# VainF/Diff-Pruning

Measured on AMD Instinct MI355X. Metric: importance-scored images/sec (UNet fwd+bwd+|w*dL/dw|), higher is better.
Workload: dtype f32

## Files before the change

### diff-pruning_amd/csrc/norm.hip

```cpp
#include <cstdlib>
#include "dp_common.h"

#define GN_CACHE 32
#define GN_MAXCPG 64

struct GnSrc {
    const float* x1; const float* x2; int c_split; long long s1, s2;
};

__device__ __forceinline__ const float* gn_chan_ptr(const GnSrc& s, int n, int c, int HW) {
    return (c < s.c_split) ? s.x1 + (long long)n * s.s1 + (long long)c * HW
                           : s.x2 + (long long)n * s.s2 + (long long)(c - s.c_split) * HW;
}

__global__ __launch_bounds__(256) void gn_fwd_kernel(GnSrc src, const float* __restrict__ gamma, const float* __restrict__ beta,
                                                     int C, int HW, int G, float eps, int silu, float* __restrict__ y,
                                                     long long y_img_stride, float* __restrict__ stats, DpDrop drop) {
    __shared__ float red[4];
    const int n = blockIdx.x / G;
    const int g = blockIdx.x - n * G;
    const int cpg = C / G;
    const int cnt = cpg * HW;
    const long long didx0 = ((drop.n_off + n) * C + (long long)g * cpg) * HW;
    const int tid = threadIdx.x;
// ... 38 lines not shown
    }
    const float var = dp_block_sum_256(q, red) / (float)cnt;
    const float rstd = 1.0f / sqrtf(var + eps);
    if (tid == 0) {
        stats[(long long)blockIdx.x * 2 + 0] = mean;
        stats[(long long)blockIdx.x * 2 + 1] = rstd;
    }
    float* yb = y + (long long)n * y_img_stride + (long long)c_base * HW;
    if (cached) {
#pragma unroll
        for (int i = 0; i < GN_CACHE; ++i) {
            const int e = tid + 256 * i;
            if (e < cnt) {
                const int c = c_base + e / HW;
                float v = (xr[i] - mean) * rstd * gamma[c] + beta[c];
                if (silu) v = dp_silu(v);
                if (drop.thr24) v *= dp_drop1(drop, didx0 + e);
                yb[e] = v;
            }
        }
    } else {
        for (int e = tid; e < cnt; e += 256) {
            const int cl = e / HW;
            const int c = c_base + cl;
            float v = (gn_chan_ptr(src, n, c, HW)[e - cl * HW] - mean) * rstd * gamma[c] + beta[c];
            if (silu) v = dp_silu(v);
            if (drop.thr24) v *= dp_drop1(drop, didx0 + e);
            yb[e] = v;
        }
    }
}

template <int NI>
__global__ __launch_bounds__(256) void gn_fwd_vec4_kernel(GnSrc src, const float* __restrict__ gamma,
                                                          const float* __restrict__ beta, int C, int HW, int G, float eps,
                                                          int silu, float* __restrict__ y, long long y_img_stride,
                                                          float* __restrict__ stats, DpDrop drop) {
    __shared__ float red[4];
    const int n = blockIdx.x / G;
    const int g = blockIdx.x - n * G;
    const int cpg = C / G;
    const int cnt4 = cpg * HW / 4;
    const long long didx0 = ((drop.n_off + n) * C + (long long)g * cpg) * HW;
    const int HW4 = HW / 4;
    const int tid = threadIdx.x;
    constexpr bool cached = NI > 0;
    constexpr int NC = NI > 0 ? NI : 1;
    const int c_base = g * cpg;
    float4 xr[NC];
    float gac[NC], bec[NC];
    float s = 0.f;
    if (cached) {
#pragma unroll
        for (int i = 0; i < NC; ++i) {
            const int e = tid + 256 * i;
            const int ec = e < cnt4 ? e : cnt4 - 1;
            const int cl = ec / HW4;
            xr[i] = reinterpret_cast<const float4*>(gn_chan_ptr(src, n, c_base + cl, HW))[ec - cl * HW4];
            gac[i] = gamma[c_base + cl];
            bec[i] = beta[c_base + cl];
        }
#pragma unroll
        for (int i = 0; i < NC; ++i) {
            if (tid + 256 * i >= cnt4) xr[i] = make_float4(0.f, 0.f, 0.f, 0.f);
            const float4 v = xr[i];
            s += (v.x + v.y) + (v.z + v.w);
        }
    } else {
        for (int e = tid; e < cnt4; e += 256) {
            const int cl = e / HW4;
            const float4 v = reinterpret_cast<const float4*>(gn_chan_ptr(src, n, c_base + cl, HW))[e - cl * HW4];
// ... 20 lines not shown
            q += (a * a + b * b) + (c * c + d * d);
        }
    }
    const float var = dp_block_sum_256(q, red) / (float)(cnt4 * 4);
    const float rstd = 1.0f / sqrtf(var + eps);
    if (tid == 0) {
        stats[(long long)blockIdx.x * 2 + 0] = mean;
        stats[(long long)blockIdx.x * 2 + 1] = rstd;
    }
    float4* yb = reinterpret_cast<float4*>(y + (long long)n * y_img_stride + (long long)c_base * HW);
    auto apply = [&](float4 v, float ga, float be, int e4) {
        float4 o;
        o.x = (v.x - mean) * rstd * ga + be;
        o.y = (v.y - mean) * rstd * ga + be;
        o.z = (v.z - mean) * rstd * ga + be;
        o.w = (v.w - mean) * rstd * ga + be;
        if (silu) { o.x = dp_silu(o.x); o.y = dp_silu(o.y); o.z = dp_silu(o.z); o.w = dp_silu(o.w); }
        if (drop.thr24) { const float4 m = dp_drop4(drop, didx0 + 4ll * e4); o.x *= m.x; o.y *= m.y; o.z *= m.z; o.w *= m.w; }
        return o;
    };
    if (cached) {
#pragma unroll
        for (int i = 0; i < NC; ++i) {
            const int e = tid + 256 * i;
            if (e < cnt4) yb[e] = apply(xr[i], gac[i], bec[i], e);
        }
    } else {
        for (int e = tid; e < cnt4; e += 256) {
            const int cl = e / HW4;
            yb[e] = apply(reinterpret_cast<const float4*>(gn_chan_ptr(src, n, c_base + cl, HW))[e - cl * HW4], gamma[c_base + cl],
                          beta[c_base + cl], e);
        }
    }
}

#define GN_WAVE_NV 8
template <int NV>
__global__ __launch_bounds__(256) void gn_fwd_wave_kernel(GnSrc src, const float* __restrict__ gamma,
                                                          const float* __restrict__ beta, int C, int HW, int G, float eps,
                                                          int silu, float* __restrict__ y, long long y_img_stride,
                                                          float* __restrict__ stats, DpDrop drop, int NG) {
    const int wid = blockIdx.x * 4 + (threadIdx.x >> 6);
    if (wid >= NG) return;
    const int lane = threadIdx.x & 63;
    const int n = wid / G;
    const int g = wid - n * G;
    const int cpg = C / G;
    const int HW4 = HW / 4;
    const int cnt4 = cpg * HW4;
    const int c_base = g * cpg;
    const long long didx0 = ((drop.n_off + n) * C + (long long)g * cpg) * HW;
    float4 xr[NV];
    float ga[NV], be[NV];
    float s = 0.f;
#pragma unroll
    for (int i = 0; i < NV; ++i) {
        const int e = lane + 64 * i;
        const int ec = e < cnt4 ? e : cnt4 - 1;
        const int cl = ec / HW4;
        xr[i] = reinterpret_cast<const float4*>(gn_chan_ptr(src, n, c_base + cl, HW))[ec - cl * HW4];
        ga[i] = gamma[c_base + cl];
        be[i] = beta[c_base + cl];
    }
#pragma unroll
    for (int i = 0; i < NV; ++i) {
        if (lane + 64 * i >= cnt4) xr[i] = make_float4(0.f, 0.f, 0.f, 0.f);
// ... 29 lines not shown
            o.w = (v.w - mean) * rstd * ga[i] + be[i];
            if (silu) { o.x = dp_silu(o.x); o.y = dp_silu(o.y); o.z = dp_silu(o.z); o.w = dp_silu(o.w); }
            if (drop.thr24) { const float4 m = dp_drop4(drop, didx0 + 4ll * e); o.x *= m.x; o.y *= m.y; o.z *= m.z; o.w *= m.w; }
            yb[e] = o;
        }
    }
}

extern "C" int dp_groupnorm_silu_fwd(const float* x1, const float* x2, int c_split, long long x1_img_stride,
                                     long long x2_img_stride, const float* gamma, const float* beta, int N, int C, int HW,
                                     int G, float eps, int silu, float* y, long long y_img_stride, float* stats,
                                     const dp_dropout* drop, void* stream) {
    if (N <= 0 || C <= 0) return 0;
    if (C % G) return (int)hipErrorInvalidValue;
    const DpDrop dd = dp_drop_host(drop);
    GnSrc s{x1, x2, x2 ? c_split : C, x1_img_stride, x2_img_stride};
    const bool vec4 = (HW % 4 == 0) && (x1_img_stride % 4 == 0) && (x2_img_stride % 4 == 0) && (y_img_stride % 4 == 0) &&
                      (((uintptr_t)x1 | (uintptr_t)x2 | (uintptr_t)y) % 16 == 0);
    static const bool no_wave = getenv("DP_NO_GN_WAVE") != nullptr;
    if (vec4 && !no_wave && (long long)(C / G) * HW <= 256 * GN_WAVE_NV && N * G >= 1024)
    {
        const int cnt4 = (C / G) * (HW / 4);
#define GN_FWD_WAVE(NV_) DP_LAUNCH((gn_fwd_wave_kernel<NV_>), dim3((N * G + 3) / 4), dim3(256), 0, (hipStream_t)stream, s, gamma, \
                                   beta, C, HW, G, eps, silu, y, y_img_stride, stats, dd, N * G)
        if (cnt4 <= 64) GN_FWD_WAVE(1);
        else if (cnt4 <= 128) GN_FWD_WAVE(2);
        else if (cnt4 <= 256) GN_FWD_WAVE(4);
        else GN_FWD_WAVE(8);
#undef GN_FWD_WAVE
    }
    else if (vec4) {
        const long long cnt4 = (long long)(C / G) * (HW / 4);
#define GN_FWD_V4(NI_) DP_LAUNCH((gn_fwd_vec4_kernel<NI_>), dim3(N * G), dim3(256), 0, (hipStream_t)stream, s, gamma, beta, C, HW, G, \
                                 eps, silu, y, y_img_stride, stats, dd)
        if (cnt4 <= 256) GN_FWD_V4(1);
        else if (cnt4 <= 512) GN_FWD_V4(2);
        else if (cnt4 <= 1024) GN_FWD_V4(4);
        else if (cnt4 <= 2048) GN_FWD_V4(8);
        else GN_FWD_V4(0);
#undef GN_FWD_V4
    }
    else
        DP_LAUNCH(gn_fwd_kernel, dim3(N * G), dim3(256), 0, (hipStream_t)stream, s, gamma, beta, C, HW, G, eps, silu,
                           y, y_img_stride, stats, dd);
    return DP_LAUNCH_CHECK();
}

__global__ __launch_bounds__(256) void gn_bwd_kernel(GnSrc src, const float* __restrict__ gamma, const float* __restrict__ beta,
                                                     const float* __restrict__ stats, const float* __restrict__ dz,
                                                     long long dz_img_stride, int C, int HW, int G, int silu,
                                                     float* __restrict__ dx, long long dx_img_stride,
                                                     const float* __restrict__ add1, long long add1_s,
                                                     const float* __restrict__ add2, long long add2_s,
                                                     float* __restrict__ pws, DpDrop drop, float* __restrict__ rows) {
    __shared__ float s1[GN_MAXCPG], s2[GN_MAXCPG];
    const int n = blockIdx.x / G;
    const int g = blockIdx.x - n * G;
    const int cpg = C / G;
    const int tid = threadIdx.x;
    const int lane = tid & 63;
    const int wave = tid >> 6;
    const int c_base = g * cpg;
    const float mean = stats[(long long)blockIdx.x * 2 + 0];
    const float rstd = stats[(long long)blockIdx.x * 2 + 1];
    const float* dzb = dz + (long long)n * dz_img_stride;
    const long long didx0 = ((drop.n_off + n) * C + c_base) * (long long)HW;

// ... 28 lines not shown
        b += ga * s2[cl];
    }
    const float invM = 1.0f / (float)(cpg * HW);
    a *= invM;
    b *= invM;

    float* dxb = dx + (long long)n * dx_img_stride + (long long)c_base * HW;
    const float* a1b = add1 ? add1 + (long long)n * add1_s + (long long)c_base * HW : nullptr;
    const float* a2b = add2 ? add2 + (long long)n * add2_s + (long long)c_base * HW : nullptr;
    for (int cl = wave; cl < cpg; cl += 4) {
        const int c = c_base + cl;
        const float* xp = gn_chan_ptr(src, n, c, HW);
        const float ga = gamma[c], be = beta[c];
        float rs = 0.f;
        for (int i = lane; i < HW; i += 64) {
            const int e = cl * HW + i;
            const float xh = (xp[i] - mean) * rstd;
            float d = dzb[(long long)c_base * HW + e];
            if (drop.thr24) d *= dp_drop1(drop, didx0 + e);
            if (silu) d *= dp_silu_grad(xh * ga + be);
            float v = rstd * (ga * d - a - xh * b);
            if (a1b) v += a1b[e];
            if (a2b) v += a2b[e];
            dxb[e] = v;
            rs += v;
        }
        if (rows) {
            rs = dp_wave_sum(rs);
            if (lane == 0) rows[(long long)n * C + c] = rs;
        }
    }
}

__global__ __launch_bounds__(256) void gn_bwd_vec4_kernel(GnSrc src, const float* __restrict__ gamma,
                                                          const float* __restrict__ beta, const float* __restrict__ stats,
                                                          const float* __restrict__ dz, long long dz_img_stride, int C,
                                                          int HW, int G, int silu, float* __restrict__ dx,
                                                          long long dx_img_stride, const float* __restrict__ add1,
                                                          long long add1_s, const float* __restrict__ add2, long long add2_s,
                                                          float* __restrict__ pws, DpDrop drop, float* __restrict__ rows) {
    __shared__ float s1[GN_MAXCPG], s2[GN_MAXCPG];
    const int n = blockIdx.x / G;
    const int g = blockIdx.x - n * G;
    const int cpg = C / G;
    const int tid = threadIdx.x;
    const int lane = tid & 63;
    const int wave = tid >> 6;
    const int c_base = g * cpg;
    const int HW4 = HW / 4;
    const float mean = stats[(long long)blockIdx.x * 2 + 0];
    const float rstd = stats[(long long)blockIdx.x * 2 + 1];
    const float* dzb = dz + (long long)n * dz_img_stride;
    const long long didx0 = ((drop.n_off + n) * C + c_base) * (long long)HW;
    auto dyv = [&](float4 xv, float4 dv, float ga, float be, float4& xh, long long e4) {
        xh.x = (xv.x - mean) * rstd; xh.y = (xv.y - mean) * rstd; xh.z = (xv.z - mean) * rstd; xh.w = (xv.w - mean) * rstd;
        if (drop.thr24) { const float4 m = dp_drop4(drop, didx0 + 4 * e4); dv.x *= m.x; dv.y *= m.y; dv.z *= m.z; dv.w *= m.w; }
        if (silu) {
            dv.x *= dp_silu_grad(xh.x * ga + be); dv.y *= dp_silu_grad(xh.y * ga + be);
            dv.z *= dp_silu_grad(xh.z * ga + be); dv.w *= dp_silu_grad(xh.w * ga + be);
        }
        return dv;
    };
    for (int cl = wave; cl < cpg; cl += 4) {
        const int c = c_base + cl;
        const float4* xp = reinterpret_cast<const float4*>(gn_chan_ptr(src, n, c, HW));
        const float4* dp = reinterpret_cast<const float4*>(dzb + (long long)c * HW);
        const float ga = gamma[c], be = beta[c];
        float a1 = 0.f, a2 = 0.f;
        for (int i = lane; i < HW4; i += 64) {
            float4 xh;
            const float4 d = dyv(xp[i], dp[i], ga, be, xh, (long long)cl * HW4 + i);
            a1 += (d.x + d.y) + (d.z + d.w);
            a2 += (d.x * xh.x + d.y * xh.y) + (d.z * xh.z + d.w * xh.w);
        }
        a1 = dp_wave_sum(a1);
        a2 = dp_wave_sum(a2);
        if (lane == 0) {
            s1[cl] = a1;
            s2[cl] = a2;
            pws[((long long)n * C + c) * 2 + 0] = a1;
            pws[((long long)n * C + c) * 2 + 1] = a2;
        }
    }
    __syncthreads();
    float a = 0.f, b = 0.f;
    for (int cl = 0; cl < cpg; ++cl) {
        const float ga = gamma[c_base + cl];
        a += ga * s1[cl];
        b += ga * s2[cl];
    }
    const float invM = 1.0f / (float)(cpg * HW);
    a *= invM;
    b *= invM;
    float4* dxb = reinterpret_cast<float4*>(dx + (long long)n * dx_img_stride + (long long)c_base * HW);
    const float4* dzc = reinterpret_cast<const float4*>(dzb + (long long)c_base * HW);
// ... 313 lines not shown
                                         add2_img_stride) % 4 == 0) &&
                      (((uintptr_t)x1 | (uintptr_t)x2 | (uintptr_t)dz | (uintptr_t)dx | (uintptr_t)add1 | (uintptr_t)add2) % 16 == 0);
    static const bool no_wave = getenv("DP_NO_GN_WAVE") != nullptr;
    const int HW4 = HW / 4;
    if (vec4 && !no_wave && HW4 >= 1 && HW4 <= 64 && (HW4 & (HW4 - 1)) == 0 && (long long)(C / G) * HW <= 256 * GN_WAVE_NV &&
        N * G >= 1024)
    {
        const int cnt4 = (C / G) * HW4;
#define GN_BWD_WAVE(NV_, A1_, A2_) DP_LAUNCH((gn_bwd_wave_kernel<NV_, A1_, A2_>), dim3((N * G + 3) / 4), dim3(256), 0,       \
                                             (hipStream_t)stream, s, gamma, beta, stats, dz, dz_img_stride, C, HW, G, silu, dx,  \
                                             dx_img_stride, add1, add1_img_stride, add2, add2_img_stride, pws, dd, rows, N * G)
#define GN_BWD_WAVE_A(NV_) do { if (add1 && add2) GN_BWD_WAVE(NV_, true, true); else if (add1) GN_BWD_WAVE(NV_, true, false);   \
                                else if (add2) GN_BWD_WAVE(NV_, false, true); else GN_BWD_WAVE(NV_, false, false); } while (0)
        if (cnt4 <= 64) GN_BWD_WAVE_A(1);
        else if (cnt4 <= 128) GN_BWD_WAVE_A(2);
        else if (cnt4 <= 256) GN_BWD_WAVE_A(4);
        else GN_BWD_WAVE_A(8);
#undef GN_BWD_WAVE_A
#undef GN_BWD_WAVE
    }
    else if (vec4 && HW4 <= 256 && C / G <= 8 && !getenv("DP_NO_GN_CACHE")) {
#define GN_BWD_C(NCH_, A1_, A2_) DP_LAUNCH((gn_bwd_vec4c_kernel<NCH_, A1_, A2_>), dim3(N * G), dim3(256), 0, (hipStream_t)stream, s,  \
                                           gamma, beta, stats, dz, dz_img_stride, C, HW, G, silu, dx, dx_img_stride, add1,           \
                                           add1_img_stride, add2, add2_img_stride, pws, dd, rows)
#define GN_BWD_C_A(NCH_) do { if (add1 && add2) GN_BWD_C(NCH_, true, true); else if (add1) GN_BWD_C(NCH_, true, false);              \
                              else if (add2) GN_BWD_C(NCH_, false, true); else GN_BWD_C(NCH_, false, false); } while (0)
        if (C / G <= 4) GN_BWD_C_A(1);
        else GN_BWD_C_A(2);
#undef GN_BWD_C_A
#undef GN_BWD_C
    } else if (vec4)
        DP_LAUNCH(gn_bwd_vec4_kernel, dim3(N * G), dim3(256), 0, (hipStream_t)stream, s, gamma, beta, stats, dz,
                           dz_img_stride, C, HW, G, silu, dx, dx_img_stride, add1, add1_img_stride, add2, add2_img_stride,
                           pws, dd, rows);
    else
        DP_LAUNCH(gn_bwd_kernel, dim3(N * G), dim3(256), 0, (hipStream_t)stream, s, gamma, beta, stats, dz,
                           dz_img_stride, C, HW, G, silu, dx, dx_img_stride, add1, add1_img_stride, add2, add2_img_stride,
                           pws, dd, rows);
    return DP_LAUNCH_CHECK();
}

__global__ __launch_bounds__(256) void gn_split_part_fwd_kernel(GnSrc src, int C, int HW, int S, float* __restrict__ part) {
    __shared__ float red[4];
    const int nc = blockIdx.x, sl = blockIdx.y;
    const int n = nc / C, c = nc - n * C;
    const int len4 = HW / S / 4;
    const float4* xp = reinterpret_cast<const float4*>(gn_chan_ptr(src, n, c, HW)) + (long long)sl * len4;
    float s = 0.f, q = 0.f, mean;
    if (len4 <= 1024) {
        float4 xr[4];
#pragma unroll
        for (int k = 0; k < 4; ++k) {
            const int i = threadIdx.x + 256 * k;
            xr[k] = xp[i < len4 ? i : len4 - 1];
        }
#pragma unroll
        for (int k = 0; k < 4; ++k) {
            if (threadIdx.x + 256 * k >= len4) xr[k] = make_float4(0.f, 0.f, 0.f, 0.f);
            s += (xr[k].x + xr[k].y) + (xr[k].z + xr[k].w);
        }
        mean = dp_block_sum_256(s, red) / (float)(len4 * 4);
#pragma unroll
        for (int k = 0; k < 4; ++k) {
            if (threadIdx.x + 256 * k < len4) {
                const float a = xr[k].x - mean, b = xr[k].y - mean, cc = xr[k].z - mean, d = xr[k].w - mean;
                q += (a * a + b * b) + (cc * cc + d * d);
            }
// ... 392 lines not shown
```

### diff-pruning_amd/csrc/ups9.hip

```cpp
#include "dp_common.h"

typedef float f32x2 __attribute__((ext_vector_type(2)));

#define U9_RSRC_FLAGS 0x00020000
#define U9_OOB 0x80000000u

__device__ __forceinline__ __amdgpu_buffer_rsrc_t u9_rsrc(const float* base, unsigned bytes) {
    return __builtin_amdgcn_make_buffer_rsrc((void*)base, 0, (int)bytes, U9_RSRC_FLAGS);
}
__device__ __forceinline__ float u9_bload(__amdgpu_buffer_rsrc_t r, unsigned byte_off) {
    asm volatile("" : "+v"(byte_off));
    return __builtin_bit_cast(float, __builtin_amdgcn_raw_buffer_load_b32(r, (int)byte_off, 0, 0));
}
__device__ __forceinline__ f32x4 u9_bload4(__amdgpu_buffer_rsrc_t r, unsigned byte_off) {
    asm volatile("" : "+v"(byte_off));
    return __builtin_bit_cast(f32x4, __builtin_amdgcn_raw_buffer_load_b128(r, (int)byte_off, 0, 0));
}

template <int BM, int BN, int KC, int WM, int WN, int OCC>
__global__ __launch_bounds__(256, OCC) void ups9_dgrad_kernel(const dp_ups9_params p) {
    constexpr int TM = BM / (32 * WM), TN = BN / (32 * WN);
    constexpr int KT = 9 * KC;
    constexpr int PT = BN * KC / 256;
    constexpr int KSTEP = 256 / BN;
    constexpr int MCH = BM / 4;
    constexpr int ACH = KT * MCH;
    constexpr int NA = (ACH + 255) / 256;
    static_assert(WM * WN == 4 && TM >= 1 && TN >= 1 && PT >= 1 && (BN * KC) % 256 == 0 && KT % 2 == 0 && BN <= 256, "tile");
    __shared__ __attribute__((aligned(16))) float As[KT * BM];
    __shared__ __attribute__((aligned(16))) float Ts[KT * BN];

    const int tid = threadIdx.x;
    const int lane = tid & 63;
    const int wave = __builtin_amdgcn_readfirstlane(tid >> 6);
    const int li = lane & 31, lk = lane >> 5;
    const int wm0 = (wave / WN) * (TM * 32), wn0 = (wave % WN) * (TN * 32);
    const int H = p.H, W = p.W, HW = H * W, W2 = 2 * W, HW4 = 4 * HW;
    const int K = p.K, M = p.M;
    const int NPIX = p.N * HW;
    const int MT = (M + BM - 1) / BM;
    const int PTILES = (NPIX + BN - 1) / BN;
    int mt, ptile;
    {
        const int b = blockIdx.x;
        if (!(PTILES & 7)) {
            const int xcd = b & 7, slot = b >> 3;
            mt = slot % MT;
            ptile = (slot / MT) * 8 + xcd;
        } else {
            mt = b % MT;
            ptile = b / MT;
        }
    }
    const int m0 = mt * BM, px0 = ptile * BN;

    const int ppix = tid % BN, pk0 = tid / BN;
    int pbase;
    bool pvalid, top, bot, left, right;
    {
        const int pixel = px0 + ppix;
        pvalid = pixel < NPIX;
        const int n = pixel / HW, rem = pixel - n * HW;
        const int i = rem / W, j = rem - i * W;
        pbase = (int)(n * p.dy_img_stride) + (2 * i - 1) * W2 + (2 * j - 1);
        top = i > 0, bot = i < H - 1, left = j > 0, right = j < W - 1;
    }
    const __amdgpu_buffer_rsrc_t rA = u9_rsrc(p.U, p.u_bytes);
    const __amdgpu_buffer_rsrc_t rB = u9_rsrc(p.dy, p.dy_bytes);

    float pr[PT][16];
    f32x4 ar[NA];
    auto load_tile = [&](int k0) {
#pragma unroll
        for (int j = 0; j < NA; ++j) {
            const int e = tid + 256 * j;
            const int kk = e / MCH, m = m0 + 4 * (e % MCH);
            const int tap = kk / KC, k = k0 + kk % KC;
            const bool v = e < ACH && m < p.ldu && k < K;
            ar[j] = u9_bload4(rA, v ? (unsigned)((((8 - tap) * K + k) * p.ldu + m) * 4) : U9_OOB);
        }
#pragma unroll
        for (int q = 0; q < PT; ++q) {
            const int k = k0 + pk0 + KSTEP * q;
            const bool ok = pvalid && k < K;
            const int off0 = pbase + k * HW4;
#pragma unroll
            for (int r = 0; r < 4; ++r) {
                const bool rok = ok && (r == 0 ? top : r == 3 ? bot : true);
#pragma unroll
                for (int c = 0; c < 4; ++c) {
                    const bool v = rok && (c == 0 ? left : c == 3 ? right : true);
                    pr[q][4 * r + c] = u9_bload(rB, v ? (unsigned)((off0 + r * W2 + c) * 4) : U9_OOB);
                }
            }
        }
    };
    auto store_tile = [&]() {
#pragma unroll
        for (int j = 0; j < NA; ++j)
            if (NA * 256 == ACH || tid + 256 * j < ACH) *(f32x4*)&As[(tid + 256 * j) * 4] = ar[j];
#pragma unroll
        for (int q = 0; q < PT; ++q) {
            const float* d = pr[q];
            float t[3][4];
#pragma unroll
            for (int c = 0; c < 4; ++c) {
                t[0][c] = d[12 + c] - d[4 + c];
                t[1][c] = d[4 + c] + d[8 + c];
                t[2][c] = d[c] - d[8 + c];
            }
            const int kc = pk0 + KSTEP * q;
#pragma unroll
            for (int a = 0; a < 3; ++a) {
                Ts[((3 * a + 0) * KC + kc) * BN + ppix] = t[a][3] - t[a][1];
                Ts[((3 * a + 1) * KC + kc) * BN + ppix] = t[a][1] + t[a][2];
                Ts[((3 * a + 2) * KC + kc) * BN + ppix] = t[a][0] - t[a][2];
            }
        }
    };

    f32x16 acc[TM][TN];
#pragma unroll
    for (int tm = 0; tm < TM; ++tm)
#pragma unroll
        for (int tn = 0; tn < TN; ++tn)
#pragma unroll
            for (int r = 0; r < 16; ++r) acc[tm][tn][r] = 0.f;

    const int nIter = (K + KC - 1) / KC;
    load_tile(0);
    for (int it = 0; it < nIter; ++it) {
        __syncthreads();
        store_tile();
        __syncthreads();
        if (it + 1 < nIter) load_tile((it + 1) * KC);
        float a[2][TM], b[2][TN];
        auto frag = [&](int ks, float (&fa)[TM], float (&fb)[TN]) {
            const int kk = ks * 2 + lk;
#pragma unroll
            for (int tm = 0; tm < TM; ++tm) fa[tm] = As[kk * BM + wm0 + tm * 32 + li];
#pragma unroll
            for (int tn = 0; tn < TN; ++tn) fb[tn] = Ts[kk * BN + wn0 + tn * 32 + li];
        };
        frag(0, a[0], b[0]);
#pragma unroll
        for (int ks = 0; ks < KT / 2; ++ks) {
            const int cur = ks & 1;
            if (ks + 1 < KT / 2) frag(ks + 1, a[cur ^ 1], b[cur ^ 1]);
            __builtin_amdgcn_sched_barrier(0);
#pragma unroll
            for (int tm = 0; tm < TM; ++tm)
#pragma unroll
                for (int tn = 0; tn < TN; ++tn)
                    acc[tm][tn] = __builtin_amdgcn_mfma_f32_32x32x2f32(a[cur][tm], b[cur][tn], acc[tm][tn], 0, 0, 0);
            __builtin_amdgcn_sched_barrier(0);
        }
    }

#pragma unroll
    for (int tn = 0; tn < TN; ++tn) {
        const int pixel = px0 + wn0 + tn * 32 + li;
        if (pixel >= NPIX) continue;
        const int n = pixel / HW, rem = pixel - n * HW;
        float* o = p.dx + (long long)n * p.dx_img_stride + rem;
#pragma unroll
        for (int tm = 0; tm < TM; ++tm)
#pragma unroll
            for (int r = 0; r < 16; ++r) {
                const int row = m0 + wm0 + tm * 32 + (r & 3) + 8 * (r >> 2) + 4 * lk;
                if (row < M) {
                    float* q = o + (long long)row * HW;
                    *q = p.accumulate ? *q + acc[tm][tn][r] : acc[tm][tn][r];
                }
            }
    }
}

static const int u9_bn[3] = {32, 64, 128};

extern "C" int dp_ups9_dgrad_supported(const dp_ups9_params* pp) {
    const dp_ups9_params& p = *pp;
// ... 5 lines not shown
    if (npix >= (1ll << 29)) return 0;
    if (9ll * p.K * p.ldu * 4 != (long long)p.u_bytes || p.u_bytes >= 0x80000000u) return 0;
    if (p.dy_img_stride < 4 * HW * p.K || p.dx_img_stride < HW * p.M) return 0;
    const long long dy_need = ((p.N - 1) * p.dy_img_stride + 4 * HW * p.K) * 4;
    if ((long long)p.dy_bytes < dy_need || p.dy_bytes >= 0x80000000u) return 0;
    const long long blocks = ((npix + u9_bn[p.tile] - 1) / u9_bn[p.tile]) * ((p.M + 127) / 128);
    if (blocks >= (1ll << 31)) return 0;
    return 1;
}

extern "C" int dp_ups9_dgrad(const dp_ups9_params* pp, void* stream) {
    if (!dp_ups9_dgrad_supported(pp)) return (int)hipErrorInvalidValue;
    const dp_ups9_params& p = *pp;
    const long long npix = (long long)p.N * p.H * p.W;
    const int bn = u9_bn[p.tile];
    const dim3 grid((unsigned)(((npix + bn - 1) / bn) * ((p.M + 127) / 128)));
    hipStream_t st = (hipStream_t)stream;
    if (p.tile == 0)      DP_LAUNCH((ups9_dgrad_kernel<128, 32, 8, 4, 1, 2>), grid, dim3(256), 0, st, p);
    else if (p.tile == 1) DP_LAUNCH((ups9_dgrad_kernel<128, 64, 4, 2, 2, 3>), grid, dim3(256), 0, st, p);
    else                  DP_LAUNCH((ups9_dgrad_kernel<128, 128, 4, 2, 2, 2>), grid, dim3(256), 0, st, p);
    return DP_LAUNCH_CHECK();
}

template <int BM, int BN, int KC, int OCC>
__global__ __launch_bounds__(256, OCC) void ups9_fwd_kernel(const dp_ups9_fwd_params p) {
    constexpr int WN = BN / 32;
    constexpr int KT = 9 * KC;
    constexpr int PT = BN * KC / 256;
    constexpr int KSTEP = 256 / BN;
    constexpr int MCH = BM / 4;
    constexpr int ACH = KT * MCH;
    constexpr int NA = (ACH + 255) / 256;
    constexpr int NS = 9 * KC / 2;
    static_assert((BM / 32) * WN == 4 && PT >= 1 && BN * KC % 256 == 0 && KC % 2 == 0 && BM % 32 == 0 && BN % 32 == 0, "tile");
    __shared__ __attribute__((aligned(16))) float As[KT * BM];
    __shared__ __attribute__((aligned(16))) float Vs[KT * BN];

    const int tid = threadIdx.x;
    const int lane = tid & 63;
    const int wave = __builtin_amdgcn_readfirstlane(tid >> 6);
    const int li = lane & 31, lk = lane >> 5;
    const int wm0 = (wave / WN) * 32, wn0 = (wave % WN) * 32;
    const int H = p.H, W = p.W, HW = H * W;
    const int K = p.K, M = p.M;
    const int NPIX = p.N * HW;
    const int MT = (M + BM - 1) / BM;
    const int PTILES = (NPIX + BN - 1) / BN;
    int mt, ptile;
    {
        const int b = blockIdx.x;
        if (!(PTILES & 7)) {
            const int xcd = b & 7, slot = b >> 3;
            mt = slot % MT;
            ptile = (slot / MT) * 8 + xcd;
        } else {
            mt = b % MT;
            ptile = b / MT;
        }
    }
    const int m0 = mt * BM, px0 = ptile * BN;

    const int ppix = tid % BN, pk0 = tid / BN;
    int pbase;
    bool pvalid, top, bot, left, right;
    {
        const int pixel = px0 + ppix;
        pvalid = pixel < NPIX;
        const int n = pixel / HW, rem = pixel - n * HW;
        const int i = rem / W, j = rem - i * W;
        pbase = (int)(n * p.x_img_stride) + (i - 1) * W + (j - 1);
        top = i > 0, bot = i < H - 1, left = j > 0, right = j < W - 1;
    }
    const __amdgpu_buffer_rsrc_t rA = u9_rsrc(p.U, p.u_bytes);
    const __amdgpu_buffer_rsrc_t rB = u9_rsrc(p.x, p.x_bytes);

    float pr[PT][9];
    f32x4 ar[NA];
    auto load_tile = [&](int k0) {
#pragma unroll
        for (int j = 0; j < NA; ++j) {
            const int e = tid + 256 * j;
            const int kk = e / MCH, m = m0 + 4 * (e % MCH);
            const int tap = kk / KC, k = k0 + kk % KC;
            const bool v = e < ACH && m < p.ldu && k < K;
            ar[j] = u9_bload4(rA, v ? (unsigned)(((tap * K + k) * p.ldu + m) * 4) : U9_OOB);
        }
#pragma unroll
        for (int q = 0; q < PT; ++q) {
            const int k = k0 + pk0 + KSTEP * q;
            const bool ok = pvalid && k < K;
            const int off0 = pbase + k * HW;
#pragma unroll
            for (int r = 0; r < 3; ++r) {
                const bool rok = ok && (r == 0 ? top : r == 2 ? bot : true);
#pragma unroll
                for (int c = 0; c < 3; ++c) {
                    const bool v = rok && (c == 0 ? left : c == 2 ? right : true);
                    pr[q][3 * r + c] = u9_bload(rB, v ? (unsigned)((off0 + r * W + c) * 4) : U9_OOB);
                }
            }
        }
    };
    auto store_tile = [&]() {
#pragma unroll
        for (int j = 0; j < NA; ++j)
            if (NA * 256 == ACH || tid + 256 * j < ACH) *(f32x4*)&As[(tid + 256 * j) * 4] = ar[j];
#pragma unroll
        for (int q = 0; q < PT; ++q) {
            const float* d = pr[q];
            float t[3][3];
#pragma unroll
            for (int c = 0; c < 3; ++c) {
                t[0][c] = d[c] - d[3 + c];
                t[1][c] = d[3 + c];
                t[2][c] = d[6 + c] - d[3 + c];
            }
            const int kc = pk0 + KSTEP * q;
#pragma unroll
            for (int a = 0; a < 3; ++a) {
                Vs[((3 * a + 0) * KC + kc) * BN + ppix] = t[a][0] - t[a][1];
                Vs[((3 * a + 1) * KC + kc) * BN + ppix] = t[a][1];
                Vs[((3 * a + 2) * KC + kc) * BN + ppix] = t[a][2] - t[a][1];
            }
        }
    };

    f32x16 acc[9];
#pragma unroll
    for (int t = 0; t < 9; ++t)
#pragma unroll
        for (int r = 0; r < 16; ++r) acc[t][r] = 0.f;

    const int nIter = (K + KC - 1) / KC;
    load_tile(0);
    for (int it = 0; it < nIter; ++it) {
        __syncthreads();
        store_tile();
        __syncthreads();
        if (it + 1 < nIter) load_tile((it + 1) * KC);
        float a[3], b[3];
        auto frag = [&](int s, float& fa, float& fb) {
            const int kk = (s % 9) * KC + (s / 9) * 2 + lk;
            fa = As[kk * BM + wm0 + li];
            fb = Vs[kk * BN + wn0 + li];
        };
        frag(0, a[0], b[0]);
        frag(1, a[1], b[1]);
#pragma unroll
        for (int s = 0; s < NS; ++s) {
            if (s + 2 < NS) frag(s + 2, a[(s + 2) % 3], b[(s + 2) % 3]);
            __builtin_amdgcn_sched_barrier(0);
            acc[s % 9] = __builtin_amdgcn_mfma_f32_32x32x2f32(a[s % 3], b[s % 3], acc[s % 9], 0, 0, 0);
            __builtin_amdgcn_sched_barrier(0);
        }
    }

    const int pixel = px0 + wn0 + li;
    if (pixel >= NPIX) return;
    const int n = pixel / HW, rem = pixel - n * HW;
    const int i = rem / W, j = rem - i * W;
    float* o = p.y + (long long)n * p.y_img_stride + (long long)(2 * i) * (2 * W) + 2 * j;
#pragma unroll
    for (int r = 0; r < 16; ++r) {
        const int row = m0 + wm0 + (r & 3) + 8 * (r >> 2) + 4 * lk;
        if (row < M) {
            const float bv = p.bias ? p.bias[row] : 0.f;
            const float c0 = acc[0][r] + acc[3][r], c1 = acc[1][r] + acc[4][r], c2 = acc[2][r] + acc[5][r];
            const float d0 = acc[3][r] + acc[6][r], d1 = acc[4][r] + acc[7][r], d2 = acc[5][r] + acc[8][r];
            float* q = o + (long long)row * (4 * HW);
            f32x2 y0, y1;
            y0[0] = (c0 + c1) + bv, y0[1] = (c1 + c2) + bv;
            y1[0] = (d0 + d1) + bv, y1[1] = (d1 + d2) + bv;
            *(f32x2*)q = y0;
            *(f32x2*)(q + 2 * W) = y1;
        }
    }
}

#define U9F_BM 64
#define U9F_BN 64

static bool u9f_ok(const dp_ups9_fwd_params& p) {
    if (!p.U || !p.x || !p.y || ((uintptr_t)p.U & 15) || ((uintptr_t)p.y & 7) || ((uintptr_t)p.bias & 3)) return false;
// ... 52 lines not shown
```

Measured before the change: 5097.

## Double-buffer ups9 GEMM tiles and add register-cached wide GroupNorm paths

The upsample Winograd-style dgrad kernels gain a two-stage LDS ring. Stores for the next tile and loads for the tile after it are interleaved piece by piece between MFMA steps, which removes one barrier per iteration. GroupNorm forward gets a 12-slot register-cached variant for groups too large for the existing cached paths. GroupNorm backward gets a wide body that keeps x and dz in registers across the reduction and output passes, so they are read from memory once. These changes double the LDS footprint and raise register pressure, which may reduce occupancy.

```diff
diff --git a/diff-pruning_amd/csrc/norm.hip b/diff-pruning_amd/csrc/norm.hip
--- a/diff-pruning_amd/csrc/norm.hip
+++ b/diff-pruning_amd/csrc/norm.hip
@@ -94,11 +94,9 @@
 }
 
 template <int NI>
-__global__ __launch_bounds__(256) void gn_fwd_vec4_kernel(GnSrc src, const float* __restrict__ gamma,
-                                                          const float* __restrict__ beta, int C, int HW, int G, float eps,
-                                                          int silu, float* __restrict__ y, long long y_img_stride,
-                                                          float* __restrict__ stats, DpDrop drop) {
-    __shared__ float red[4];
+__device__ __forceinline__ void gn_fwd_vec4_body(const GnSrc& src, const float* __restrict__ gamma, const float* __restrict__ beta,
+                                                 int C, int HW, int G, float eps, int silu, float* __restrict__ y,
+                                                 long long y_img_stride, float* __restrict__ stats, const DpDrop& drop, float* red) {
     const int n = blockIdx.x / G;
     const int g = blockIdx.x - n * G;
     const int cpg = C / G;
@@ -185,6 +183,19 @@
                           beta[c_base + cl], e);
         }
     }
+}
+
+#define GN_WIDE_SLOTS 12
+template <int NI>
+__global__ __launch_bounds__(256) void gn_fwd_vec4_kernel(GnSrc src, const float* __restrict__ gamma,
+                                                          const float* __restrict__ beta, int C, int HW, int G, float eps,
+                                                          int silu, float* __restrict__ y, long long y_img_stride,
+                                                          float* __restrict__ stats, DpDrop drop, int streaming) {
+    __shared__ float red[4];
+    if (NI == 0 && !streaming && (C / G) * HW / 4 <= 256 * GN_WIDE_SLOTS)
+        gn_fwd_vec4_body<GN_WIDE_SLOTS>(src, gamma, beta, C, HW, G, eps, silu, y, y_img_stride, stats, drop, red);
+    else
+        gn_fwd_vec4_body<NI>(src, gamma, beta, C, HW, G, eps, silu, y, y_img_stride, stats, drop, red);
 }
 
 #define GN_WAVE_NV 8
@@ -280,7 +291,8 @@
     else if (vec4) {
         const long long cnt4 = (long long)(C / G) * (HW / 4);
 #define GN_FWD_V4(NI_) DP_LAUNCH((gn_fwd_vec4_kernel<NI_>), dim3(N * G), dim3(256), 0, (hipStream_t)stream, s, gamma, beta, C, HW, G, \
-                                 eps, silu, y, y_img_stride, stats, dd)
+                                 eps, silu, y, y_img_stride, stats, dd, streaming)
+        const int streaming = getenv("DP_NO_GN_CACHE") != nullptr;
         if (cnt4 <= 256) GN_FWD_V4(1);
         else if (cnt4 <= 512) GN_FWD_V4(2);
         else if (cnt4 <= 1024) GN_FWD_V4(4);
@@ -375,13 +387,120 @@
     }
 }
 
-__global__ __launch_bounds__(256) void gn_bwd_vec4_kernel(GnSrc src, const float* __restrict__ gamma,
+template <int NCH, int J, class DYV>
+__device__ __forceinline__ void gn_bwd_wide_body(const GnSrc& src, const float* __restrict__ gamma, const float* __restrict__ beta,
+                                                 const DYV& dyv, float rstd, const float* dzb, int n, int C, int HW, int cpg, int c_base,
+                                                 float* __restrict__ dx, long long dx_img_stride, const float* __restrict__ add1,
+                                                 long long add1_s, const float* __restrict__ add2, long long add2_s,
+                                                 float* __restrict__ pws, float* __restrict__ rows, float* s1, float* s2) {
+    static_assert(NCH * J == GN_WIDE_SLOTS, "slots");
+    const int lane = threadIdx.x & 63;
+    const int wave = __builtin_amdgcn_readfirstlane(threadIdx.x >> 6);
+    const int HW4 = HW / 4;
+    float4 xh[NCH][J], dd[NCH][J];
+    float gak[NCH], bek[NCH];
+#pragma unroll
+    for (int k = 0; k < NCH; ++k) {
+        const int cl = wave + 4 * k;
+        if (cl < cpg) {
+            const int c = c_base + cl;
+            const float4* xp = reinterpret_cast<const float4*>(gn_chan_ptr(src, n, c, HW));
+            const float4* dp = reinterpret_cast<const float4*>(dzb + (long long)c * HW);
+            gak[k] = gamma[c];
+            bek[k] = beta[c];
+#pragma unroll
+            for (int j = 0; j < J; ++j) {
+                const int i = lane + 64 * j;
+                const int ic = i < HW4 ? i : HW4 - 1;
+                xh[k][j] = xp[ic];
+                dd[k][j] = dp[ic];
+            }
+        }
+    }
+#pragma unroll
+    for (int k = 0; k < NCH; ++k) {
+        const int cl = wave + 4 * k;
+        if (cl < cpg) {
+            const int c = c_base + cl;
+            float a1 = 0.f, a2 = 0.f;
+#pragma unroll
+            for (int j = 0; j < J; ++j) {
+                const int i = lane + 64 * j;
+                if (i < HW4) {
+                    float4 h;
+                    const float4 d = dyv(xh[k][j], dd[k][j], gak[k], bek[k], h, (long long)cl * HW4 + i);
+                    xh[k][j] = h;
+                    dd[k][j] = d;
+                    {
+#pragma clang fp contract(off)
+                        a1 += (d.x + d.y) + (d.z + d.w);
+                        a2 += (d.x * h.x + d.y * h.y) + (d.z * h.z + d.w * h.w);
+                    }
+                }
+            }
+            a1 = dp_wave_sum(a1);
+            a2 = dp_wave_sum(a2);
+            if (lane == 0) {
+                s1[cl] = a1;
+                s2[cl] = a2;
+                pws[((long long)n * C + c) * 2 + 0] = a1;
+                pws[((long long)n * C + c) * 2 + 1] = a2;
+            }
+        }
+    }
+    __syncthreads();
+    float a = 0.f, b = 0.f;
+    for (int cl = 0; cl < cpg; ++cl) {
+        const float ga = gamma[c_base + cl];
+        a += ga * s1[cl];
+        b += ga * s2[cl];
+    }
+    const float invM = 1.0f / (float)(cpg * HW);
+    a *= invM;
+    b *= invM;
+    float4* dxb = reinterpret_cast<float4*>(dx + (long long)n * dx_img_stride + (long long)c_base * HW);
+    const float4* a1b = add1 ? reinterpret_cast<const float4*>(add1 + (long long)n * add1_s + (long long)c_base * HW) : nullptr;
+    const float4* a2b = add2 ? reinterpret_cast<const float4*>(add2 + (long long)n * add2_s + (long long)c_base * HW) : nullptr;
+    const float4 zero4 = make_float4(0.f, 0.f, 0.f, 0.f);
+#pragma unroll
+    for (int k = 0; k < NCH; ++k) {
+        const int cl = wave + 4 * k;
+        if (cl < cpg) {
+            const float ga = gak[k];
+            float r = 0.f;
+#pragma unroll
+            for (int j = 0; j < J; ++j) {
+                const int i = lane + 64 * j;
+                const int e = cl * HW4 + (i < HW4 ? i : HW4 - 1);
+                float4 t1 = zero4, t2 = zero4;
+                if (a1b) t1 = a1b[e];
+                if (a2b) t2 = a2b[e];
+                if (i < HW4) {
+                    const float4 d = dd[k][j], h = xh[k][j];
+                    float4 v;
+                    v.x = rstd * (ga * d.x - a - h.x * b) + t1.x + t2.x;
+                    v.y = rstd * (ga * d.y - a - h.y * b) + t1.y + t2.y;
+                    v.z = rstd * (ga * d.z - a - h.z * b) + t1.z + t2.z;
+                    v.w = rstd * (ga * d.w - a - h.w * b) + t1.w + t2.w;
+                    dxb[e] = v;
+                    r += (v.x + v.y) + (v.z + v.w);
+                }
+            }
+            if (rows) {
+                r = dp_wave_sum(r);
+                if (lane == 0) rows[(long long)n * C + c_base + cl] = r;
+            }
+        }
+    }
+}
+
+__global__ __launch_bounds__(256, 4) void gn_bwd_vec4_kernel(GnSrc src, const float* __restrict__ gamma,
                                                           const float* __restrict__ beta, const float* __restrict__ stats,
                                                           const float* __restrict__ dz, long long dz_img_stride, int C,
                                                           int HW, int G, int silu, float* __restrict__ dx,
                                                           long long dx_img_stride, const float* __restrict__ add1,
                                                           long long add1_s, const float* __restrict__ add2, long long add2_s,
-                                                          float* __restrict__ pws, DpDrop drop, float* __restrict__ rows) {
+                                                          float* __restrict__ pws, DpDrop drop, float* __restrict__ rows, int streaming) {
     __shared__ float s1[GN_MAXCPG], s2[GN_MAXCPG];
     const int n = blockIdx.x / G;
     const int g = blockIdx.x - n * G;
@@ -404,6 +523,27 @@
         }
         return dv;
     };
+    if (!streaming && !drop.thr24 && HW4 <= 256) {
+        const int J = (HW4 + 63) >> 6;
+        if (((cpg + 3) >> 2) * J <= GN_WIDE_SLOTS) {
+            auto dyv0 = [&](float4 xv, float4 dv, float ga, float be, float4& xh, long long) {
+                xh.x = (xv.x - mean) * rstd; xh.y = (xv.y - mean) * rstd; xh.z = (xv.z - mean) * rstd; xh.w = (xv.w - mean) * rstd;
+                if (silu) {
+                    dv.x *= dp_silu_grad(xh.x * ga + be); dv.y *= dp_silu_grad(xh.y * ga + be);
+                    dv.z *= dp_silu_grad(xh.z * ga + be); dv.w *= dp_silu_grad(xh.w * ga + be);
+                }
+                return dv;
+            };
+#define GN_BWD_WIDE(NCH_, J_) gn_bwd_wide_body<NCH_, J_>(src, gamma, beta, dyv0, rstd, dzb, n, C, HW, cpg, c_base, dx, dx_img_stride, add1, \
+                                                         add1_s, add2, add2_s, pws, rows, s1, s2)
+            if (J == 1) GN_BWD_WIDE(12, 1);
+            else if (J == 2) GN_BWD_WIDE(6, 2);
+            else if (J == 3) GN_BWD_WIDE(4, 3);
+            else GN_BWD_WIDE(3, 4);
+#undef GN_BWD_WIDE
+            return;
+        }
+    }
     for (int cl = wave; cl < cpg; cl += 4) {
         const int c = c_base + cl;
         const float4* xp = reinterpret_cast<const float4*>(gn_chan_ptr(src, n, c, HW));
@@ -783,7 +923,7 @@
     } else if (vec4)
         DP_LAUNCH(gn_bwd_vec4_kernel, dim3(N * G), dim3(256), 0, (hipStream_t)stream, s, gamma, beta, stats, dz,
                            dz_img_stride, C, HW, G, silu, dx, dx_img_stride, add1, add1_img_stride, add2, add2_img_stride,
-                           pws, dd, rows);
+                           pws, dd, rows, getenv("DP_NO_GN_CACHE") != nullptr ? 1 : 0);
     else
         DP_LAUNCH(gn_bwd_kernel, dim3(N * G), dim3(256), 0, (hipStream_t)stream, s, gamma, beta, stats, dz,
                            dz_img_stride, C, HW, G, silu, dx, dx_img_stride, add1, add1_img_stride, add2, add2_img_stride,
diff --git a/diff-pruning_amd/csrc/ups9.hip b/diff-pruning_amd/csrc/ups9.hip
--- a/diff-pruning_amd/csrc/ups9.hip
+++ b/diff-pruning_amd/csrc/ups9.hip
@@ -16,6 +16,8 @@
     asm volatile("" : "+v"(byte_off));
     return __builtin_bit_cast(f32x4, __builtin_amdgcn_raw_buffer_load_b128(r, (int)byte_off, 0, 0));
 }
+
+constexpr int u9_stages(int bytes) { return 2 * 2 * bytes <= 160 * 1024 ? 2 : 1; }
 
 template <int BM, int BN, int KC, int WM, int WN, int OCC>
 __global__ __launch_bounds__(256, OCC) void ups9_dgrad_kernel(const dp_ups9_params p) {
@@ -26,9 +28,13 @@
     constexpr int MCH = BM / 4;
     constexpr int ACH = KT * MCH;
     constexpr int NA = (ACH + 255) / 256;
+    constexpr int NST = u9_stages(KT * (BM + BN) * 4);
+    constexpr int NCHUNK = NA + 3 * PT;
+    constexpr int CH0 = KT / 2 - NCHUNK - 1;
     static_assert(WM * WN == 4 && TM >= 1 && TN >= 1 && PT >= 1 && (BN * KC) % 256 == 0 && KT % 2 == 0 && BN <= 256, "tile");
-    __shared__ __attribute__((aligned(16))) float As[KT * BM];
-    __shared__ __attribute__((aligned(16))) float Ts[KT * BN];
+    static_assert(NST == 1 || CH0 >= 1, "ring: more store pieces than k-steps");
+    __shared__ __attribute__((aligned(16))) float As[NST * KT * BM];
+    __shared__ __attribute__((aligned(16))) float Ts[NST * KT * BN];
 
     const int tid = threadIdx.x;
     const int lane = tid & 63;
@@ -70,30 +76,32 @@
 
     float pr[PT][16];
     f32x4 ar[NA];
+    auto load_a = [&](int j, int k0) {
+        const int e = tid + 256 * j;
+        const int kk = e / MCH, m = m0 + 4 * (e % MCH);
+        const int tap = kk / KC, k = k0 + kk % KC;
+        const bool v = e < ACH && m < p.ldu && k < K;
+        ar[j] = u9_bload4(rA, v ? (unsigned)((((8 - tap) * K + k) * p.ldu + m) * 4) : U9_OOB);
+    };
+    auto load_patch = [&](int q, int k0) {
+        const int k = k0 + pk0 + KSTEP * q;
+        const bool ok = pvalid && k < K;
+        const int off0 = pbase + k * HW4;
+#pragma unroll
+        for (int r = 0; r < 4; ++r) {
+            const bool rok = ok && (r == 0 ? top : r == 3 ? bot : true);
+#pragma unroll
+            for (int c = 0; c < 4; ++c) {
+                const bool v = rok && (c == 0 ? left : c == 3 ? right : true);
+                pr[q][4 * r + c] = u9_bload(rB, v ? (unsigned)((off0 + r * W2 + c) * 4) : U9_OOB);
+            }
+        }
+    };
     auto load_tile = [&](int k0) {
 #pragma unroll
-        for (int j = 0; j < NA; ++j) {
-            const int e = tid + 256 * j;
-            const int kk = e / MCH, m = m0 + 4 * (e % MCH);
-            const int tap = kk / KC, k = k0 + kk % KC;
-            const bool v = e < ACH && m < p.ldu && k < K;
-            ar[j] = u9_bload4(rA, v ? (unsigned)((((8 - tap) * K + k) * p.ldu + m) * 4) : U9_OOB);
-        }
-#pragma unroll
-        for (int q = 0; q < PT; ++q) {
-            const int k = k0 + pk0 + KSTEP * q;
-            const bool ok = pvalid && k < K;
-            const int off0 = pbase + k * HW4;
-#pragma unroll
-            for (int r = 0; r < 4; ++r) {
-                const bool rok = ok && (r == 0 ? top : r == 3 ? bot : true);
-#pragma unroll
-                for (int c = 0; c < 4; ++c) {
-                    const bool v = rok && (c == 0 ? left : c == 3 ? right : true);
-                    pr[q][4 * r + c] = u9_bload(rB, v ? (unsigned)((off0 + r * W2 + c) * 4) : U9_OOB);
-                }
-            }
-        }
+        for (int j = 0; j < NA; ++j) load_a(j, k0);
+#pragma unroll
+        for (int q = 0; q < PT; ++q) load_patch(q, k0);
     };
     auto store_tile = [&]() {
 #pragma unroll
@@ -118,6 +126,25 @@
             }
         }
     };
+    auto load_piece = [&](int c, int k0) {
+        if (c < NA) load_a(c, k0);
+        else if ((c - NA) % 3 == 2) load_patch((c - NA) / 3, k0);
+    };
+    auto store_piece = [&](int c, float* Ad, float* Td) {
+        if (c < NA) {
+            if (NA * 256 == ACH || tid + 256 * c < ACH) *(f32x4*)&Ad[(tid + 256 * c) * 4] = ar[c];
+        } else {
+            const int q = (c - NA) / 3, a = (c - NA) % 3;
+            const float* d = pr[q];
+            float t[4];
+#pragma unroll
+            for (int cc = 0; cc < 4; ++cc) t[cc] = a == 0 ? d[12 + cc] - d[4 + cc] : a == 1 ? d[4 + cc] + d[8 + cc] : d[cc] - d[8 + cc];
+            const int kc = pk0 + KSTEP * q;
+            Td[((3 * a + 0) * KC + kc) * BN + ppix] = t[3] - t[1];
+            Td[((3 * a + 1) * KC + kc) * BN + ppix] = t[1] + t[2];
+            Td[((3 * a + 2) * KC + kc) * BN + ppix] = t[0] - t[2];
+        }
+    };
 
     f32x16 acc[TM][TN];
 #pragma unroll
@@ -129,24 +156,39 @@
 
     const int nIter = (K + KC - 1) / KC;
     load_tile(0);
+    if (NST == 2) {
+#pragma unroll
+        for (int c = 0; c < NCHUNK; ++c) store_piece(c, As, Ts);
+        load_tile(KC);
+    }
     for (int it = 0; it < nIter; ++it) {
         __syncthreads();
-        store_tile();
-        __syncthreads();
-        if (it + 1 < nIter) load_tile((it + 1) * KC);
+        if (NST == 1) {
+            store_tile();
+            __syncthreads();
+        }
+        const float* Ac = NST == 2 ? As + (it & 1) * (KT * BM) : As;
+        const float* Tc = NST == 2 ? Ts + (it & 1) * (KT * BN) : Ts;
+        float* An = NST == 2 ? As + ((it + 1) & 1) * (KT * BM) : As;
+        float* Tn = NST == 2 ? Ts + ((it + 1) & 1) * (KT * BN) : Ts;
+        if (NST == 1 && it + 1 < nIter) load_tile((it + 1) * KC);
         float a[2][TM], b[2][TN];
         auto frag = [&](int ks, float (&fa)[TM], float (&fb)[TN]) {
             const int kk = ks * 2 + lk;
 #pragma unroll
-            for (int tm = 0; tm < TM; ++tm) fa[tm] = As[kk * BM + wm0 + tm * 32 + li];
-#pragma unroll
-            for (int tn = 0; tn < TN; ++tn) fb[tn] = Ts[kk * BN + wn0 + tn * 32 + li];
+            for (int tm = 0; tm < TM; ++tm) fa[tm] = Ac[kk * BM + wm0 + tm * 32 + li];
+#pragma unroll
+            for (int tn = 0; tn < TN; ++tn) fb[tn] = Tc[kk * BN + wn0 + tn * 32 + li];
         };
         frag(0, a[0], b[0]);
 #pragma unroll
         for (int ks = 0; ks < KT / 2; ++ks) {
             const int cur = ks & 1;
             if (ks + 1 < KT / 2) frag(ks + 1, a[cur ^ 1], b[cur ^ 1]);
+            if (NST == 2 && ks >= CH0 && ks < CH0 + NCHUNK) {
+                store_piece(ks - CH0, An, Tn);
+                load_piece(ks - CH0, (it + 2) * KC);
+            }
             __builtin_amdgcn_sched_barrier(0);
 #pragma unroll
             for (int tm = 0; tm < TM; ++tm)
@@ -218,9 +260,13 @@
     constexpr int ACH = KT * MCH;
     constexpr int NA = (ACH + 255) / 256;
     constexpr int NS = 9 * KC / 2;
+    constexpr int NST = u9_stages(KT * (BM + BN) * 4);
+    constexpr int NCHUNK = NA + 3 * PT;
+    constexpr int CH0 = NS - NCHUNK - 2;
     static_assert((BM / 32) * WN == 4 && PT >= 1 && BN * KC % 256 == 0 && KC % 2 == 0 && BM % 32 == 0 && BN % 32 == 0, "tile");
-    __shared__ __attribute__((aligned(16))) float As[KT * BM];
-    __shared__ __attribute__((aligned(16))) float Vs[KT * BN];
+    static_assert(NST == 1 || CH0 >= 1, "ring: more store pieces than MFMA steps");
+    __shared__ __attribute__((aligned(16))) float As[NST * KT * BM];
+    __shared__ __attribute__((aligned(16))) float Vs[NST * KT * BN];
 
     const int tid = threadIdx.x;
     const int lane = tid & 63;
@@ -262,30 +308,32 @@
 
     float pr[PT][9];
     f32x4 ar[NA];
+    auto load_a = [&](int j, int k0) {
+        const int e = tid + 256 * j;
+        const int kk = e / MCH, m = m0 + 4 * (e % MCH);
+        const int tap = kk / KC, k = k0 + kk % KC;
+        const bool v = e < ACH && m < p.ldu && k < K;
+        ar[j] = u9_bload4(rA, v ? (unsigned)(((tap * K + k) * p.ldu + m) * 4) : U9_OOB);
+    };
+    auto load_patch = [&](int q, int k0) {
+        const int k = k0 + pk0 + KSTEP * q;
+        const bool ok = pvalid && k < K;
+        const int off0 = pbase + k * HW;
+#pragma unroll
+        for (int r = 0; r < 3; ++r) {
+            const bool rok = ok && (r == 0 ? top : r == 2 ? bot : true);
+#pragma unroll
+            for (int c = 0; c < 3; ++c) {
+                const bool v = rok && (c == 0 ? left : c == 2 ? right : true);
+                pr[q][3 * r + c] = u9_bload(rB, v ? (unsigned)((off0 + r * W + c) * 4) : U9_OOB);
+            }
+        }
+    };
     auto load_tile = [&](int k0) {
 #pragma unroll
-        for (int j = 0; j < NA; ++j) {
-            const int e = tid + 256 * j;
-            const int kk = e / MCH, m = m0 + 4 * (e % MCH);
-            const int tap = kk / KC, k = k0 + kk % KC;
-            const bool v = e < ACH && m < p.ldu && k < K;
-            ar[j] = u9_bload4(rA, v ? (unsigned)(((tap * K + k) * p.ldu + m) * 4) : U9_OOB);
-        }
-#pragma unroll
-        for (int q = 0; q < PT; ++q) {
-            const int k = k0 + pk0 + KSTEP * q;
-            const bool ok = pvalid && k < K;
-            const int off0 = pbase + k * HW;
-#pragma unroll
-            for (int r = 0; r < 3; ++r) {
-                const bool rok = ok && (r == 0 ? top : r == 2 ? bot : true);
-#pragma unroll
-                for (int c = 0; c < 3; ++c) {
-                    const bool v = rok && (c == 0 ? left : c == 2 ? right : true);
-                    pr[q][3 * r + c] = u9_bload(rB, v ? (unsigned)((off0 + r * W + c) * 4) : U9_OOB);
-                }
-            }
-        }
+        for (int j = 0; j < NA; ++j) load_a(j, k0);
+#pragma unroll
+        for (int q = 0; q < PT; ++q) load_patch(q, k0);
     };
     auto store_tile = [&]() {
 #pragma unroll
@@ -310,6 +358,25 @@
             }
         }
     };
+    auto load_piece = [&](int c, int k0) {
+        if (c < NA) load_a(c, k0);
+        else if ((c - NA) % 3 == 2) load_patch((c - NA) / 3, k0);
+    };
+    auto store_piece = [&](int c, float* Ad, float* Vd) {
+        if (c < NA) {
+            if (NA * 256 == ACH || tid + 256 * c < ACH) *(f32x4*)&Ad[(tid + 256 * c) * 4] = ar[c];
+        } else {
+            const int q = (c - NA) / 3, a = (c - NA) % 3;
+            const float* d = pr[q];
+            float t[3];
+#pragma unroll
+            for (int cc = 0; cc < 3; ++cc) t[cc] = a == 0 ? d[cc] - d[3 + cc] : a == 1 ? d[3 + cc] : d[6 + cc] - d[3 + cc];
+            const int kc = pk0 + KSTEP * q;
+            Vd[((3 * a + 0) * KC + kc) * BN + ppix] = t[0] - t[1];
+            Vd[((3 * a + 1) * KC + kc) * BN + ppix] = t[1];
+            Vd[((3 * a + 2) * KC + kc) * BN + ppix] = t[2] - t[1];
+        }
+    };
 
     f32x16 acc[9];
 #pragma unroll
@@ -319,22 +386,37 @@
 
     const int nIter = (K + KC - 1) / KC;
     load_tile(0);
+    if (NST == 2) {
+#pragma unroll
+        for (int c = 0; c < NCHUNK; ++c) store_piece(c, As, Vs);
+        load_tile(KC);
+    }
     for (int it = 0; it < nIter; ++it) {
         __syncthreads();
-        store_tile();
-        __syncthreads();
-        if (it + 1 < nIter) load_tile((it + 1) * KC);
+        if (NST == 1) {
+            store_tile();
+            __syncthreads();
+        }
+        const float* Ac = NST == 2 ? As + (it & 1) * (KT * BM) : As;
+        const float* Vc = NST == 2 ? Vs + (it & 1) * (KT * BN) : Vs;
+        float* An = NST == 2 ? As + ((it + 1) & 1) * (KT * BM) : As;
+        float* Vn = NST == 2 ? Vs + ((it + 1) & 1) * (KT * BN) : Vs;
+        if (NST == 1 && it + 1 < nIter) load_tile((it + 1) * KC);
         float a[3], b[3];
         auto frag = [&](int s, float& fa, float& fb) {
             const int kk = (s % 9) * KC + (s / 9) * 2 + lk;
-            fa = As[kk * BM + wm0 + li];
-            fb = Vs[kk * BN + wn0 + li];
+            fa = Ac[kk * BM + wm0 + li];
+            fb = Vc[kk * BN + wn0 + li];
         };
         frag(0, a[0], b[0]);
         frag(1, a[1], b[1]);
 #pragma unroll
         for (int s = 0; s < NS; ++s) {
             if (s + 2 < NS) frag(s + 2, a[(s + 2) % 3], b[(s + 2) % 3]);
+            if (NST == 2 && s >= CH0 && s < CH0 + NCHUNK) {
+                store_piece(s - CH0, An, Vn);
+                load_piece(s - CH0, (it + 2) * KC);
+            }
             __builtin_amdgcn_sched_barrier(0);
             acc[s % 9] = __builtin_amdgcn_mfma_f32_32x32x2f32(a[s % 3], b[s % 3], acc[s % 9], 0, 0, 0);
             __builtin_amdgcn_sched_barrier(0);
```

Measured after the change: 5130, median of 6. Within noise of the previous version (+0.7%).
